# yanivw12/gs2mesh

Hardware: AMD Instinct MI355X
Metric: stereo-pair renders/sec + TSDF Mvoxel-updates/sec (higher is better)
Workload: dtype f32

## Files before the change

gs2mesh_amd/csrc/raster_api.hip:

```cpp
#include <stdarg.h>
#include <stdio.h>
#include <stdlib.h>
#include <string.h>

#include <string>
#include <vector>

#include "../../include/gs2mesh_amd.h"
#include "device_memory.h"
#include "raster_internal.h"

static thread_local std::string g_err;
void gs2m_set_error(const char* fmt, ...) {
    char buf[1024];
    va_list ap;
    va_start(ap, fmt);
    vsnprintf(buf, sizeof(buf), fmt, ap);
    va_end(ap);
    g_err = buf;
}
extern "C" const char* gs2m_last_error(void) { return g_err.c_str(); }
extern "C" int gs2m_version(void) { return GS2M_VERSION; }

#define GS2M_SORT_CLASSES_API 3
#define GS2M_MAX_STATUS 64

struct gs2m_raster {
    int device = 0;
    int opt_exact_cull = 0, opt_blend = 4, opt_debug = 0, opt_timing = 0, opt_tile_rows = 1, opt_pair_batch = 0;
    int opt_bin_workgroups = 256, opt_bin_wg_threads = 1024, opt_blend_mode = 2;
    int opt_blend_profile = 0;
    int opt_project_shared = 0;
    int opt_bin_lane_tiles = 4;
    DeviceBuffer<unsigned long long> d_blend_prof;
    EventPool events;
    DeviceBuffer<CamUniform> d_cams;
    DeviceBuffer<float4> d_recs;
    DeviceBuffer<unsigned long long> d_tilemask;
    DeviceBuffer<float> d_shpack;
    const float* pack_src = nullptr;
    const float* pack_src_rest = nullptr;
    int pack_P = 0;
    DeviceBuffer<float> d_pk_xyz, d_pk_scales, d_pk_rots, d_pk_opac;
    DeviceBuffer<int> d_order, d_rank;
    const float* model_src[4] = {nullptr, nullptr, nullptr, nullptr};
    bool model_packed = false;
    bool hint_valid = false;
    bool last_packed = false;
    const int* run_rank = nullptr;
    DeviceBuffer<unsigned> d_hist;
    DeviceBuffer<unsigned> d_tile_count, d_tile_start;
    DeviceBuffer<unsigned> d_sort_lists;
    DeviceBuffer<unsigned long long> d_keys, d_tmp;
    unsigned inst_cap = 0;
    DeviceBuffer<ViewStatus> d_status;
    PinnedBuffer<ViewStatus> h_status;
    DeviceBuffer<float> d_bw_rows;
    DeviceBuffer<unsigned> d_bw_offset;
    DeviceBuffer<unsigned> d_bw_blocks;
    DeviceBuffer<unsigned long long> d_bw_total;
    unsigned long long bw_last_rows = 0;
    bool fw_valid = false;
    int fw_P = 0, fw_W = 0, fw_H = 0, fw_tile_rows = 1;
    int last_P = 0, last_nv = 0, last_tiles = 0, last_views_total = 0;
    unsigned last_cap = 0;
};

extern "C" int gs2m_raster_create(gs2m_raster** out, int device) {
    if (!out) {
        gs2m_set_error("gs2m_raster_create: out is NULL");
        return 1;
    }
    GS2M_HIPCHK(hipSetDevice(device));
    gs2m_raster* r = new gs2m_raster();
    r->device = device;
    const size_t n_status = GS2M_MAX_STATUS + 1;
    if (r->d_cams.reserve_exact(GS2M_MAX_PASS_VIEWS) || r->d_status.reserve_exact(n_status) || r->h_status.reserve(n_status) ||
        hipMemset(r->d_status.get(), 0, sizeof(ViewStatus) * n_status) != hipSuccess) {
        gs2m_set_error("gs2m_raster_create: allocation failed");
        delete r;
        return 1;
    }
    memset(r->h_status.get(), 0, sizeof(ViewStatus) * n_status);
    *out = r;
    return 0;
}

extern "C" int gs2m_raster_destroy(gs2m_raster* r) {
    delete r;
    return 0;
}

extern "C" int gs2m_raster_set_option(gs2m_raster* r, int option, int value) {
    if (!r) {
        gs2m_set_error("null handle");
        return 1;
    }
    switch (option) {
        case GS2M_OPT_EXACT_TILE_CULL:
            if (value < 0 || value > 2) {
                gs2m_set_error("GS2M_OPT_EXACT_TILE_CULL must be 0, 1 or 2");
                return 1;
            }
            r->opt_exact_cull = value;
            return 0;
        case GS2M_OPT_BLEND_VARIANT:
            if (value != 0 && value != 4) {
                gs2m_set_error("GS2M_OPT_BLEND_VARIANT must be 0 or 4");
                return 1;
            }
            r->opt_blend = value;
            return 0;
        case GS2M_OPT_TILE_ROWS:
            if (value != 1 && value != 2) {
                gs2m_set_error("GS2M_OPT_TILE_ROWS must be 1 or 2");
                return 1;
// ... 95 lines not shown
        return 1;
    }
    if (instances > 0 && (unsigned)instances > r->inst_cap) r->inst_cap = (unsigned)instances;
    if (r->inst_cap < 1024) r->inst_cap = 1024;
    if (r->d_keys.reserve((size_t)nv * r->inst_cap)) return 1;
    if (r->d_tmp.reserve((size_t)nv * r->inst_cap)) return 1;
    return 0;
}

static int dbg_check(gs2m_raster* r, hipStream_t st, const char* what) {
    if (!r->opt_debug) return 0;
    hipError_t e = hipStreamSynchronize(st);
    if (e == hipSuccess) e = hipGetLastError();
    if (e != hipSuccess) {
        gs2m_set_error("[debug] after %s: %s", what, hipGetErrorString(e));
        return 1;
    }
    return 0;
}

static const char* const kStageRange[GS2M_N_STAGES] = {"gs2m:project", "gs2m:hist_colscan", "gs2m:tile_scan", "gs2m:scatter",
                                                        "gs2m:sort_tiles", "gs2m:blend", "gs2m:count_tiles"};
static StageTimer stage_timer(gs2m_raster* r, hipStream_t st, int stage) {
    return StageTimer(r->events, r->opt_timing != 0, st, stage, kStageRange[stage]);
}

static int run_views(gs2m_raster* r, const GaussIn& g, int nv, int pairs, int W, int H, float* out_color,
                     unsigned char* out_rgb8, int* out_radii, int status_slot, hipStream_t st, const CamUniform* host_cams) {
    const int nvt = nv * pairs;
    const int gx = (W + GS2M_TILE - 1) / GS2M_TILE, gy = (H + GS2M_TILE - 1) / GS2M_TILE;
    const int gys = (gy + r->opt_tile_rows - 1) / r->opt_tile_rows;
    const int tiles = gx * gys;
    int hint[3] = {-1, -1, -1};
    int interleave = 1;
    const ViewStatus* hs = r->h_status.get() + 1 + status_slot;
    if (r->hint_valid && r->last_tiles == tiles && r->last_nv == nvt) {
        unsigned nr_max = 0;
        for (int c = 0; c < 3; ++c) {
            unsigned m = 0;
            for (int v = 0; v < nvt; ++v) {
                const unsigned x = hs[v].n_class[c];
                m = x > m ? x : m;
            }
            hint[c] = m > 0x3fffffffu ? -1 : (int)m;
        }
        for (int v = 0; v < nvt; ++v) {
            const unsigned x = hs[v].num_rendered;
            nr_max = x > nr_max ? x : nr_max;
        }
        if (nr_max > 0u && nr_max <= 0x3fffffffu) interleave = (size_t)nr_max >= (size_t)800 * (size_t)tiles;
    }
    int chunk, n_wg;
    geometry(r, g.P, &chunk, &n_wg, pairs);
    int wg_threads = (gs2m_count_threads(chunk, r->opt_bin_wg_threads) + 63) / 64 * 64;
    while (wg_threads > 64 && (gs2m_scatter_lds_bytes(nv, tiles, wg_threads) > 160 * 1024 || gs2m_count_lds_bytes(nv, tiles, wg_threads) > 160 * 1024))
        wg_threads = (wg_threads / 2 + 63) / 64 * 64;
    const size_t lds = gs2m_scatter_lds_bytes(nv, tiles, wg_threads);
    const size_t lds_p = gs2m_count_lds_bytes(nv, tiles, wg_threads);
    if (lds > 160 * 1024 || lds_p > 160 * 1024) {
        gs2m_set_error("image %dx%d: %d views x %d tiles do not fit the 160 KiB LDS tile cursors", W, H, nv, tiles);
        return 1;
    }
    if (r->inst_cap == 0) {
        int64_t guess = (int64_t)g.P * 4;
        if (guess < 65536) guess = 65536;
        r->inst_cap = (unsigned)(guess > 0xfffffff0ll ? 0xfffffff0ll : guess);
    }
    if (gs2m_raster_reserve(r, g.P, nvt, W, H, 0)) return 1;
    const unsigned cap = r->inst_cap;
    const GeomRecs recs{r->d_recs.get(), r->d_recs.get() + 2 * (size_t)nvt * (size_t)g.P};
    const int cull_arg_p = r->opt_exact_cull, cull_arg_s = r->opt_exact_cull;
    {
        StageTimer tm = stage_timer(r, st, GS2M_STAGE_PROJECT);
        gs2m_launch_project(nv, pairs, st, g, r->d_cams.get(), recs, out_radii, cull_arg_p, host_cams, r->opt_project_shared);
    }
    if (dbg_check(r, st, "project")) return 1;
    {
        StageTimer tm = stage_timer(r, st, GS2M_STAGE_COUNT);
        if (gs2m_launch_count_tiles(nv, pairs, n_wg, wg_threads, lds_p, st, recs, g.P, r->d_cams.get(), chunk, r->d_hist.get(), r->d_tilemask.get(),
                                    cull_arg_p, g.ids != nullptr, r->opt_bin_lane_tiles))
            return 1;
    }
    if (dbg_check(r, st, "count_tiles")) return 1;
    {
        StageTimer tm = stage_timer(r, st, GS2M_STAGE_COLSCAN);
        gs2m_launch_hist_colscan(st, nvt, r->d_hist.get(), n_wg, tiles, r->d_tile_count.get());
    }
    if (dbg_check(r, st, "hist_colscan")) return 1;
    {
        StageTimer tm = stage_timer(r, st, GS2M_STAGE_TILESCAN);
        gs2m_launch_tile_scan(st, nvt, r->d_tile_count.get(), r->d_tile_start.get(), tiles, gx, r->h_status.get() + 1 + status_slot, r->d_status.get(), cap, r->d_sort_lists.get());
    }
    if (dbg_check(r, st, "tile_scan")) return 1;
    {
        StageTimer tm = stage_timer(r, st, GS2M_STAGE_SCATTER);
        if (gs2m_launch_scatter(nv, pairs, n_wg, wg_threads, lds, st, recs, g.P, r->d_cams.get(), chunk, r->d_hist.get(), r->d_tile_start.get(),
                                r->d_tilemask.get(), r->d_keys.get(), cap, cull_arg_s, g.ids, g.ids != nullptr, r->opt_bin_lane_tiles))
            return 1;
    }
    if (dbg_check(r, st, "scatter")) return 1;
    {
        StageTimer tm = stage_timer(r, st, GS2M_STAGE_SORT);
        gs2m_launch_sort_tiles(st, nvt, r->d_keys.get(), r->d_tmp.get(), r->d_tile_start.get(), tiles, cap, r->d_sort_lists.get(), hint);
    }
    if (dbg_check(r, st, "sort_tiles")) return 1;
    {
        StageTimer tm = stage_timer(r, st, GS2M_STAGE_BLEND);
        if (gs2m_launch_blend(st, r->opt_blend, r->opt_tile_rows, nvt, gx, gy, r->d_keys.get(), r->d_tile_start.get(), recs, r->d_cams.get(),
                              g.P, cap, out_color, out_rgb8, g.ids ? r->run_rank : nullptr,
                              r->d_sort_lists.get() + (size_t)nvt * GS2M_SORT_CLASSES_API * (tiles + 1), r->opt_blend_mode,
                              r->opt_blend_profile ? r->d_blend_prof.get() : nullptr, interleave))
            return 1;
    }
    if (dbg_check(r, st, "blend")) return 1;
    r->last_P = g.P;
    r->hint_valid = true;
    r->last_packed = g.ids != nullptr;
    r->last_nv = nvt;
    r->last_tiles = tiles;
    r->last_cap = cap;
    return 0;
}

extern "C" int gs2m_rasterize_forward(gs2m_raster* r, int P, int D, int M, const float* background, int width,
                                      int height, const float* means3D, const float* shs,
                                      const float* colors_precomp, const float* opacities, const float* scales,
                                      float scale_modifier, const float* rotations, const float* cov3D_precomp,
                                      const float* viewmatrix, const float* projmatrix, const float* cam_pos,
                                      float tan_fovx, float tan_fovy, int prefiltered, float* out_color,
                                      int* radii, int debug, gs2m_stream stream) {
    (void)prefiltered;
    if (!r) {
        gs2m_set_error("null handle");
        return 1;
    }
    hipStream_t st = (hipStream_t)stream;
    GS2M_HIPCHK(hipSetDevice(r->device));
    if (width <= 0 || height <= 0 || !out_color) {
        gs2m_set_error("gs2m_rasterize_forward: bad image arguments");
        return 1;
    }
    if (D < 0 || D > 3) {
        gs2m_set_error("SH degree %d not in 0..3", D);
        return 1;
    }
    r->last_views_total = 1;
    r->fw_valid = false;
    if (P == 0) {
        GS2M_HIPCHK(hipMemsetAsync(out_color, 0, sizeof(float) * 3 * (size_t)width * height, st));
// ... 539 lines not shown
```

gs2mesh_amd/csrc/raster_bin.hip:

```cpp
#include "raster_sort.h"
#include "raster_internal.h"

void gs2m_launch_hist_colscan(hipStream_t st, int nv, unsigned* hist, int n_wg, int tiles, unsigned* tile_count) {
    GS2M_LAUNCH(k_hist_colscan, dim3((tiles + 63) / 64, nv), dim3(64 * GS2M_COLSCAN_SEGS), 0, st, hist, n_wg, tiles, tile_count);
}
void gs2m_launch_tile_scan(hipStream_t st, int nv, const unsigned* tile_count, unsigned* tile_start, int tiles, int gx,
                           ViewStatus* status, ViewStatus* sticky, unsigned cap, unsigned* sort_lists) {
    GS2M_LAUNCH(k_tile_scan, dim3(nv), dim3(1024), 0, st, tile_count, tile_start, tiles, gx, status, sticky, cap, sort_lists);
}
size_t gs2m_sort_lists_words(int nv, int tiles) { return (size_t)nv * (GS2M_SORT_CLASSES * (tiles + 1) + tiles); }
void gs2m_launch_sort_tiles(hipStream_t st, int nv, unsigned long long* keys, unsigned long long* tmp,
                            const unsigned* tile_start, int tiles, unsigned cap, const unsigned* sort_lists, const int* class_hint) {
    const int fold = class_hint && class_hint[0] == 0 && class_hint[1] == 0 && class_hint[2] == 0;
    GS2M_LAUNCH(k_sort_tiles_small<4>, dim3((tiles + 3) / 4, nv), dim3(256), 0, st, keys, tile_start, tiles, cap, tmp, sort_lists, fold);
    if (fold) return;
    const int full[3] = {tiles < 1024 ? tiles : 1024, tiles < 512 ? tiles : 512, tiles < 512 ? tiles : 512};
    int g[3];
    for (int c = 0; c < 3; ++c) {
        g[c] = full[c];
        if (class_hint && class_hint[c] >= 0) {
            const int want = class_hint[c] + class_hint[c] / 2 + 16;
            g[c] = want < full[c] ? want : full[c];
        }
        if (g[c] < 1) g[c] = 1;
    }
    GS2M_LAUNCH(k_sort_tiles_bucket_4096x8, dim3(g[0], nv), dim3(512), 0, st, keys, tile_start, tiles, cap, sort_lists);
    GS2M_LAUNCH(k_sort_tiles_bucket_8192x8, dim3(g[1], nv), dim3(1024), 0, st, keys, tile_start, tiles, cap, sort_lists);
    GS2M_LAUNCH(k_sort_tiles, dim3(g[2], nv), dim3(256), 0, st, keys, tmp, tile_start, tiles, cap, sort_lists);
}
```

gs2mesh_amd/csrc/raster_blend.h:

```cpp
#pragma once
#include <type_traits>
#include "raster_common.h"

GS2M_DEVICE unsigned char quantize_u8(float c) {
    float v = rintf(c * 255.0f);
    v = fminf(255.0f, fmaxf(0.0f, v));
    return (unsigned char)(int)v;
}

GS2M_KERNEL void __launch_bounds__(256)
k_blend_tile256(const unsigned long long* __restrict__ keys, const unsigned* __restrict__ tile_start,
                const GeomRecs recs, const CamUniform* __restrict__ cams, int P, unsigned cap,
                float* __restrict__ out_color, unsigned char* __restrict__ out_rgb8, const int* __restrict__ rank) {
    __shared__ float4 s_a[256];
    __shared__ float4 s_b[256];
    __shared__ float s_c[256];
    const int v = (int)blockIdx.z;
    const CamUniform& cam = cams[v];
    const int W = cam.W, H = cam.H, gx = cam.gx;
    const int tiles = gx * cam.gy;
    const int tile = (int)blockIdx.y * gx + (int)blockIdx.x;
    const int tid = (int)threadIdx.x;
    const int lx = tid & 15, ly = tid >> 4;
    const int pxi = (int)blockIdx.x * GS2M_TILE + lx, pyi = (int)blockIdx.y * GS2M_TILE + ly;
// ... 407 lines not shown
            atomicAdd(&pc[5], pt_loop);
            atomicAdd(&pc[6], pt_epi);
            atomicAdd(&pc[7], pn_batches);
            atomicAdd(&pc[8], pn_staged);
            atomicAdd(&pc[9], (unsigned long long)(r1 - r0));
        }
    }
}

template <int LROWS>
GS2M_DEVICE bool blend_slot_tile(const CamUniform& cam, const unsigned* __restrict__ order, const int v, const int xcd, const int j,
                                 int& tx, int& ty) {
    const int gx = cam.gx;
    const int ltiles = gx * ((cam.gy + LROWS - 1) / LROWS);
    const int lrows = ltiles / gx, cpr = (gx + GS2M_SCHED_CW - 1) / GS2M_SCHED_CW;
    const int nch = cpr * ((lrows + GS2M_SCHED_CH - 1) / GS2M_SCHED_CH);
    const int rank_c = (j / (GS2M_SCHED_CHUNK * LROWS)) * 8 + xcd;
    if (rank_c >= nch) return false;
    const int c = (int)order[(size_t)v * ltiles + rank_c];
    const int k = (j / LROWS) % GS2M_SCHED_CHUNK;
    const int crow = c / cpr, lx = (c - crow * cpr) * GS2M_SCHED_CW + k % GS2M_SCHED_CW;
    const int ly = crow * GS2M_SCHED_CH + k / GS2M_SCHED_CW;
    if (lx >= gx || ly >= lrows) return false;
    tx = lx;
    ty = ly * LROWS + j % LROWS;
    return ty < cam.gy;
}

template <int WPB, int LROWS, int OCC, int MODE = 0, int PROF = 0>
GS2M_KERNEL void __launch_bounds__(64 * WPB, OCC)
k_blend_wave4e(const unsigned long long* __restrict__ keys, const unsigned* __restrict__ tile_start,
               const GeomRecs recs, const CamUniform* __restrict__ cams, int P, unsigned cap,
               float* __restrict__ out_color, unsigned char* __restrict__ out_rgb8, const int* __restrict__ rank,
               const unsigned* __restrict__ order, unsigned long long* __restrict__ prof = nullptr, int nv_x = 0) {
    __shared__ float4 s_a[WPB][64 + 2], s_b[WPB][64 + 2];
    __shared__ float2 s_c[WPB][64 + 2];
    __shared__ float4 s_raw[WPB][3 * 64];
    const int tid = (int)threadIdx.x;
    const int wave = tid >> 6, lane = tid & 63;
    const int nvx = gs2m_uniform(nv_x);
    const int v = nvx > 1 ? (int)((blockIdx.x / 8u) % (unsigned)nvx) : (int)blockIdx.y;
    const unsigned bid = nvx > 1 ? (blockIdx.x / 8u / (unsigned)nvx) * 8u + blockIdx.x % 8u : blockIdx.x;
    int tx, ty;
    if (!blend_slot_tile<LROWS>(cams[v], order, v, (int)(bid % 8u), gs2m_uniform((int)(bid / 8u) * WPB + wave), tx, ty)) return;
    blend_tile<WPB, LROWS, MODE, PROF>(v, tx, ty, cams[v], keys, tile_start, recs, P, cap, out_color, out_rgb8, rank, prof, &s_a[wave][0],
                                       &s_b[wave][0], &s_c[wave][0], &s_raw[wave][0], lane);
}
```

gs2mesh_amd/csrc/raster_blend.hip:

```cpp
#include "raster_blend.h"
#include "raster_backward_blend.h"
#include "raster_internal.h"

int gs2m_launch_blend(hipStream_t st, int variant, int tile_rows, int nv, int gx, int gy, const unsigned long long* keys,
                      const unsigned* tile_start, GeomRecs recs, const CamUniform* cams, int P, unsigned cap,
                      float* out_color, unsigned char* out_rgb8, const int* rank, const unsigned* order, int mode,
                      unsigned long long* prof, int interleave_views) {
    const dim3 block(256);
    if (variant == 4) {
        const int ltiles = gx * ((gy + tile_rows - 1) / tile_rows);
        const int nch = ((gx + GS2M_SCHED_CW - 1) / GS2M_SCHED_CW) * ((ltiles / gx + GS2M_SCHED_CH - 1) / GS2M_SCHED_CH);
        const dim3 g2(8u * ((unsigned)(((nch + 7) / 8) * GS2M_SCHED_CHUNK * tile_rows + 3) / 4u), nv);
        if (mode >= 2) {
            const int nvx = interleave_views && nv > 1 ? nv : 0;
            const dim3 g1 = nvx ? dim3(g2.x * (unsigned)nv, 1) : g2;
            if (prof) {
                if (tile_rows == 2) GS2M_LAUNCH((k_blend_wave4e<4, 2, 7, 2, 1>), g1, block, 0, st, keys, tile_start, recs, cams, P, cap, out_color, out_rgb8, rank, order, prof, nvx);
                else GS2M_LAUNCH((k_blend_wave4e<4, 1, 7, 2, 1>), g1, block, 0, st, keys, tile_start, recs, cams, P, cap, out_color, out_rgb8, rank, order, prof, nvx);
                return 0;
            }
            if (mode == 3) {
                if (tile_rows == 2) GS2M_LAUNCH((k_blend_wave4e<4, 2, 7, 3>), g1, block, 0, st, keys, tile_start, recs, cams, P, cap, out_color, out_rgb8, rank, order, nullptr, nvx);
                else GS2M_LAUNCH((k_blend_wave4e<4, 1, 7, 3>), g1, block, 0, st, keys, tile_start, recs, cams, P, cap, out_color, out_rgb8, rank, order, nullptr, nvx);
                return 0;
            }
            if (tile_rows == 2) GS2M_LAUNCH((k_blend_wave4e<4, 2, 7, 2>), g1, block, 0, st, keys, tile_start, recs, cams, P, cap, out_color, out_rgb8, rank, order, nullptr, nvx);
            else GS2M_LAUNCH((k_blend_wave4e<4, 1, 7, 2>), g1, block, 0, st, keys, tile_start, recs, cams, P, cap, out_color, out_rgb8, rank, order, nullptr, nvx);
            return 0;
        }
        if (tile_rows == 2) GS2M_LAUNCH((k_blend_wave4e<4, 2, 7>), g2, block, 0, st, keys, tile_start, recs, cams, P, cap, out_color, out_rgb8, rank, order, nullptr);
        else GS2M_LAUNCH((k_blend_wave4e<4, 1, 7>), g2, block, 0, st, keys, tile_start, recs, cams, P, cap, out_color, out_rgb8, rank, order, nullptr);
        return 0;
    }
    if (variant == 0 && tile_rows == 1) {
        GS2M_LAUNCH(k_blend_tile256, dim3(gx, gy, nv), dim3(256), 0, st, keys, tile_start, recs, cams, P, cap, out_color, out_rgb8, rank);
        return 0;
    }
    gs2m_set_error("blend variant %d is not available with GS2M_OPT_TILE_ROWS %d (variants: 0 [rows 1 only], 4)", variant, tile_rows);
    return 1;
}

void gs2m_launch_blend_backward(hipStream_t st, int gx, int gy, const unsigned long long* keys, const unsigned* tile_start,
                                GeomRecs recs, const CamUniform* cams, int P, unsigned cap, const float* dL_dpix,
                                const unsigned* row_offset, float* rows, unsigned long long n_rows) {
    const int tiles = gx * gy;
    GS2M_LAUNCH((k_blend_backward<4>), dim3((tiles + 3) / 4), dim3(256), 0, st, keys, tile_start, recs, cams, P, cap, dL_dpix,
                row_offset, rows, n_rows);
}
```

gs2mesh_amd/csrc/raster_common.h:

```cpp
#pragma once
#include "platform.h"

#define GS2M_TILE 16
#define GS2M_MAX_VIEWS 2
#define GS2M_MAX_PAIRS 4
#define GS2M_MAX_PASS_VIEWS (GS2M_MAX_VIEWS * GS2M_MAX_PAIRS)
#define GS2M_SORT_LDS 4096
#ifndef GS2M_SCHED_CW
#define GS2M_SCHED_CW 4
#endif
#ifndef GS2M_SCHED_CH
#define GS2M_SCHED_CH 2
#endif
#define GS2M_SCHED_CHUNK (GS2M_SCHED_CW * GS2M_SCHED_CH)
#define GS2M_BW_ROW 12

struct CamUniform {
    float view[16];
    float proj[16];
    float campos[3];
    float tanfovx, tanfovy, focal_x, focal_y;
    int W, H, gx, gy;
    float bg[3];
    int th;
// ... 6 lines not shown
    float cc, op, r, g;
    float b, depth;
    unsigned rect0, rect1;
};
struct GeomRecs {
    float4* ab;
    float4* c;
};
GS2M_DEVICE GeomRecs gs2m_recs_at(const GeomRecs& r, size_t first) { return GeomRecs{r.ab + 2 * first, r.c + first}; }

struct GaussIn {
    const float* xyz;
    const float* scales;
    const float* rots;
    const float* opac;
    const float* shs;
    const float* shs_rest;
    const float* shs_packed;
    const float* cov3D_precomp;
    const float* colors_precomp;
    const int* ids;
    int P, D, M, raw;
    float scale_modifier;
};

GS2M_DEVICE unsigned gs2m_xcd_contiguous(unsigned bid, unsigned nwg) {
    const unsigned qq = nwg / 8u, rr = nwg % 8u, xcd = bid % 8u, idx = bid / 8u;
    return (xcd < rr ? xcd * (qq + 1u) : rr * (qq + 1u) + (xcd - rr) * qq) + idx;
}

struct ViewStatus {
    unsigned num_rendered;
    unsigned overflow;
    unsigned n_class[3];
    unsigned pad;
};
```

gs2mesh_amd/csrc/raster_internal.h:

```cpp
#pragma once
#include "api_check.h"
#include "raster_common.h"

size_t gs2m_scatter_lds_bytes(int nv, int tiles, int threads);
void gs2m_launch_project(int nv, int pairs, hipStream_t st, const GaussIn& g, CamUniform* cams, GeomRecs recs, int* radii,
                         int exact_cull, const CamUniform* host_cams, int shared_read);
int gs2m_launch_count_tiles(int nv, int pairs, int n_wg, int threads, size_t lds_bytes, hipStream_t st, GeomRecs recs, int P,
                            const CamUniform* cams, int chunk, unsigned* hist, unsigned long long* tilemask,
                            int exact_cull, int interleave, int lane_tiles);
int gs2m_count_threads(int chunk, int max_threads);
size_t gs2m_count_lds_bytes(int nv, int tiles, int threads);
int gs2m_launch_scatter(int nv, int pairs, int n_wg, int threads, size_t lds_bytes, hipStream_t st, GeomRecs recs, int P,
                        const CamUniform* cams, int chunk, const unsigned* hist, const unsigned* tile_start,
                        const unsigned long long* tilemask, unsigned long long* keys, unsigned cap, int exact_cull,
                        const int* ids, int interleave, int lane_tiles);
void gs2m_launch_pack_sh(hipStream_t st, int P, const float* shs, const float* shs_rest, float* packed, const int* order);
void gs2m_launch_pack_model(hipStream_t st, int P, const int* order, const float* xyz, const float* scales, const float* rots,
                            const float* opac, float* p_xyz, float* p_scales, float* p_rots, float* p_opac, int* rank,
                            unsigned* bad);
void gs2m_launch_mark_visible(hipStream_t st, int P, const float* xyz, const float* viewmatrix,
                              unsigned char* present);
void gs2m_launch_pack_camera(hipStream_t st, CamUniform* cams, int slot, const float* viewmatrix,
                             const float* projmatrix, const float* campos, const float* bg, float tanfovx,
                             float tanfovy, int W, int H, int th);

void gs2m_launch_hist_colscan(hipStream_t st, int nv, unsigned* hist, int n_wg, int tiles, unsigned* tile_count);
void gs2m_launch_tile_scan(hipStream_t st, int nv, const unsigned* tile_count, unsigned* tile_start, int tiles, int gx,
                           ViewStatus* status, ViewStatus* sticky, unsigned cap, unsigned* sort_lists);
size_t gs2m_sort_lists_words(int nv, int tiles);
void gs2m_launch_sort_tiles(hipStream_t st, int nv, unsigned long long* keys, unsigned long long* tmp,
                            const unsigned* tile_start, int tiles, unsigned cap, const unsigned* sort_lists, const int* class_hint);
int gs2m_launch_blend(hipStream_t st, int variant, int tile_rows, int nv, int gx, int gy, const unsigned long long* keys,
                      const unsigned* tile_start, GeomRecs recs, const CamUniform* cams, int P,
                      unsigned cap, float* out_color, unsigned char* out_rgb8, const int* rank, const unsigned* order,
                      int mode, unsigned long long* prof, int interleave_views);

struct BwOut {
    float* dL_dmean2D;
    float* dL_dconic;
    float* dL_dopacity;
    float* dL_dcolor;
    float* dL_dmean3D;
    float* dL_dcov3D;
    float* dL_dsh;
    float* dL_dscale;
    float* dL_drot;
};
void gs2m_launch_bw_row_offsets(hipStream_t st, GeomRecs recs, int P, unsigned* block_sum, unsigned* row_offset,
                                unsigned long long* total_rows);
void gs2m_launch_blend_backward(hipStream_t st, int gx, int gy, const unsigned long long* keys, const unsigned* tile_start,
                                GeomRecs recs, const CamUniform* cams, int P, unsigned cap, const float* dL_dpix,
                                const unsigned* row_offset, float* rows, unsigned long long n_rows);
void gs2m_launch_gaussian_backward(hipStream_t st, const GaussIn& g, const CamUniform* cams, GeomRecs recs,
                                   const unsigned* row_offset, const float* rows, unsigned long long n_rows, const BwOut& out);
```

gs2mesh_amd/csrc/raster_sort.h:

```cpp
#pragma once
#include <type_traits>
#include "raster_common.h"

#define GS2M_SORT_WAVE 512
#define GS2M_SORT_CLASSES 3
#define GS2M_SORT_BUCKET_CAP 8192

#define GS2M_COLSCAN_SEGS 16
GS2M_KERNEL void __launch_bounds__(1024)
k_tile_scan(const unsigned* __restrict__ tile_count, unsigned* __restrict__ tile_start, int tiles, int gx,
            ViewStatus* __restrict__ status_all, ViewStatus* __restrict__ sticky, unsigned cap, unsigned* __restrict__ sort_lists) {
    const int v = (int)blockIdx.x, n_views = (int)gridDim.x;
    ViewStatus* status = status_all + v;
    __shared__ unsigned part[16];
    __shared__ unsigned n_class[GS2M_SORT_CLASSES];
    __shared__ unsigned w_pos[64];
    __shared__ unsigned w_max;
    const int tid = (int)threadIdx.x;
    const unsigned* cnt = tile_count + (size_t)v * tiles;
    unsigned* start = tile_start + (size_t)v * (tiles + 1);
    const int per = (tiles + 1023) / 1024;
    const int lo = tid * per;
    const int hi = lo + per < tiles ? lo + per : tiles;
    unsigned* lists = sort_lists + (size_t)v * GS2M_SORT_CLASSES * (tiles + 1);
    if (tid < GS2M_SORT_CLASSES) n_class[tid] = 0u;
    if (tid < 64) w_pos[tid] = 0u;
    if (tid == 64) w_max = 0u;
    __syncthreads();
    unsigned s = 0;
    for (int i = lo; i < hi; ++i) {
        const unsigned c = cnt[i];
        s += c;
        if (c > GS2M_SORT_WAVE) {
            const int cls = c <= 4096u ? 0 : (c <= GS2M_SORT_BUCKET_CAP ? 1 : 2);
            lists[cls * (tiles + 1) + 1 + atomicAdd(&n_class[cls], 1u)] = (unsigned)i;
        }
    }
    const int lane = tid & 63, wave = tid >> 6;
    unsigned incl = s;
#pragma unroll
    for (int d = 1; d < 64; d <<= 1) {
        const unsigned y = gs2m_shfl_up(incl, d);
        if (lane >= d) incl += y;
    }
// ... 27 lines not shown
    unsigned cw[2] = {0u, 0u};
    const bool sched = nch <= 2048;
    if (sched) {
        for (int k = 0; k < 2; ++k)
            if (tid + 1024 * k < nch) {
                cw[k] = chunk_weight(tid + 1024 * k);
                atomicMax(&w_max, cw[k]);
            }
    }
    __syncthreads();
    int wsh = 0;
    while ((w_max >> wsh) > 63u) ++wsh;
    if (sched)
        for (int k = 0; k < 2; ++k)
            if (tid + 1024 * k < nch) atomicAdd(&w_pos[63u - (cw[k] >> wsh)], 1u);
    __syncthreads();
    if (tid < 64) {
        const unsigned c = w_pos[tid];
        unsigned incl2 = c;
#pragma unroll
        for (int d = 1; d < 64; d <<= 1) {
            const unsigned y = gs2m_shfl_up(incl2, d);
            if (tid >= d) incl2 += y;
        }
        w_pos[tid] = incl2 - c;
    }
    __syncthreads();
    for (int k = 0; k < 2; ++k)
        if (tid + 1024 * k < nch) order[sched ? atomicAdd(&w_pos[63u - (cw[k] >> wsh)], 1u) : (unsigned)(tid + 1024 * k)] = (unsigned)(tid + 1024 * k);
    if (!sched)
        for (int c = tid + 2048; c < nch; c += 1024) order[c] = (unsigned)c;
    if (tid < GS2M_SORT_CLASSES) {
        lists[tid * (tiles + 1)] = n_class[tid];
        status->n_class[tid] = n_class[tid];
    }
    if (tid == 1023) {
        const unsigned total = total_all;
        start[tiles] = total;
        status->num_rendered = total;
        status->overflow = total > cap ? 1u : 0u;
        if (total > cap) atomicOr(&sticky->overflow, 1u);
        atomicMax(&sticky->num_rendered, total);
    }
}

GS2M_KERNEL void __launch_bounds__(64 * GS2M_COLSCAN_SEGS)
k_hist_colscan(unsigned* __restrict__ hist, int n_wg, int tiles, unsigned* __restrict__ tile_count) {
    __shared__ unsigned seg_sum[GS2M_COLSCAN_SEGS][64];
    const int lane = (int)(threadIdx.x & 63u), seg = (int)(threadIdx.x >> 6);
    const int t = (int)blockIdx.x * 64 + lane;
    const int v = (int)blockIdx.y;
    const int per = (n_wg + GS2M_COLSCAN_SEGS - 1) / GS2M_COLSCAN_SEGS;
    const int w0 = seg * per < n_wg ? seg * per : n_wg;
    const int w1 = w0 + per < n_wg ? w0 + per : n_wg;
    unsigned* col = hist + (size_t)v * n_wg * tiles + t;
    unsigned s = 0;
    if (t < tiles) {
        int w = w0;
        for (; w + 8 <= w1; w += 8) {
            unsigned x[8];
#pragma unroll
            for (int u = 0; u < 8; ++u) x[u] = col[(size_t)(w + u) * tiles];
#pragma unroll
            for (int u = 0; u < 8; ++u) s += x[u];
        }
        for (; w < w1; ++w) s += col[(size_t)w * tiles];
    }
    seg_sum[seg][lane] = s;
    __syncthreads();
    if (t < tiles) {
        unsigned run = 0, total = 0;
#pragma unroll
        for (int k = 0; k < GS2M_COLSCAN_SEGS; ++k) {
            const unsigned x = seg_sum[k][lane];
            run += k < seg ? x : 0u;
// ... 649 lines not shown
```

gs2mesh_amd/csrc/tsdf_api.hip:

```cpp
#include <math.h>
#include <stdio.h>
#include <string.h>

#include <mutex>
#include <vector>

#include "../../include/gs2mesh_amd.h"
#include "device_memory.h"
#include "tsdf_common.h"
#include "tsdf_internal.h"

struct gs2m_tsdf {
    int device = 0;
    double voxel_length = 0, sdf_trunc = 0, unit_length = 0;
    int color_type = 1, resolution = 16, stride = 4;
    TsdfVolume V;
    struct {
        DeviceBuffer<float> tsdf, weight;
        DeviceBuffer<unsigned> rgb, stamp, touched, counters;
        DeviceBuffer<int> block_keys, hash_vals;
        DeviceBuffer<unsigned char> halo;
        DeviceBuffer<unsigned long long> hash_keys, fmask, totals;
    } vol;
    unsigned frame_id = 0;
    PinnedBuffer<unsigned> h_counters;
    PinnedBuffer<unsigned long long> h_totals;
    int n_cu = 256;
    DeviceBuffer<unsigned char> d_mc;
    const McDevTables* mc() const { return reinterpret_cast<const McDevTables*>(d_mc.get()); }
    DeviceBuffer<unsigned> d_blk_tris;
    DeviceBuffer<unsigned long long> d_ntri;
    DeviceBuffer<double> mesh_v, mesh_c;
    DeviceBuffer<int> mesh_e;
    DeviceBuffer<int> mesh_tri;
    int64_t mesh_nv = 0, mesh_nt = 0;
    ScratchArena mesh_scratch;
    int timing = 0;
    EventPool events;
    DeviceBuffer<TsdfBatchFrame> d_bframes;
    static const int kRing = 8;
    PinnedBuffer<TsdfBatchFrame> h_bframes;
    hipEvent_t ring_done[8] = {nullptr, nullptr, nullptr, nullptr, nullptr, nullptr, nullptr, nullptr};
    unsigned ring_next = 0;
    ~gs2m_tsdf() {
        for (auto e : ring_done)
            if (e) (void)hipEventDestroy(e);
    }
};

static bool invert4x4(const double* m, double* inv) {
    double a[16];
    a[0] = m[5] * m[10] * m[15] - m[5] * m[11] * m[14] - m[9] * m[6] * m[15] + m[9] * m[7] * m[14] + m[13] * m[6] * m[11] - m[13] * m[7] * m[10];
    a[4] = -m[4] * m[10] * m[15] + m[4] * m[11] * m[14] + m[8] * m[6] * m[15] - m[8] * m[7] * m[14] - m[12] * m[6] * m[11] + m[12] * m[7] * m[10];
    a[8] = m[4] * m[9] * m[15] - m[4] * m[11] * m[13] - m[8] * m[5] * m[15] + m[8] * m[7] * m[13] + m[12] * m[5] * m[11] - m[12] * m[7] * m[9];
    a[12] = -m[4] * m[9] * m[14] + m[4] * m[10] * m[13] + m[8] * m[5] * m[14] - m[8] * m[6] * m[13] - m[12] * m[5] * m[10] + m[12] * m[6] * m[9];
    a[1] = -m[1] * m[10] * m[15] + m[1] * m[11] * m[14] + m[9] * m[2] * m[15] - m[9] * m[3] * m[14] - m[13] * m[2] * m[11] + m[13] * m[3] * m[10];
    a[5] = m[0] * m[10] * m[15] - m[0] * m[11] * m[14] - m[8] * m[2] * m[15] + m[8] * m[3] * m[14] + m[12] * m[2] * m[11] - m[12] * m[3] * m[10];
    a[9] = -m[0] * m[9] * m[15] + m[0] * m[11] * m[13] + m[8] * m[1] * m[15] - m[8] * m[3] * m[13] - m[12] * m[1] * m[11] + m[12] * m[3] * m[9];
    a[13] = m[0] * m[9] * m[14] - m[0] * m[10] * m[13] - m[8] * m[1] * m[14] + m[8] * m[2] * m[13] + m[12] * m[1] * m[10] - m[12] * m[2] * m[9];
    a[2] = m[1] * m[6] * m[15] - m[1] * m[7] * m[14] - m[5] * m[2] * m[15] + m[5] * m[3] * m[14] + m[13] * m[2] * m[7] - m[13] * m[3] * m[6];
    a[6] = -m[0] * m[6] * m[15] + m[0] * m[7] * m[14] + m[4] * m[2] * m[15] - m[4] * m[3] * m[14] - m[12] * m[2] * m[7] + m[12] * m[3] * m[6];
    a[10] = m[0] * m[5] * m[15] - m[0] * m[7] * m[13] - m[4] * m[1] * m[15] + m[4] * m[3] * m[13] + m[12] * m[1] * m[7] - m[12] * m[3] * m[5];
    a[14] = -m[0] * m[5] * m[14] + m[0] * m[6] * m[13] + m[4] * m[1] * m[14] - m[4] * m[2] * m[13] - m[12] * m[1] * m[6] + m[12] * m[2] * m[5];
    a[3] = -m[1] * m[6] * m[11] + m[1] * m[7] * m[10] + m[5] * m[2] * m[11] - m[5] * m[3] * m[10] - m[9] * m[2] * m[7] + m[9] * m[3] * m[6];
    a[7] = m[0] * m[6] * m[11] - m[0] * m[7] * m[10] - m[4] * m[2] * m[11] + m[4] * m[3] * m[10] + m[8] * m[2] * m[7] - m[8] * m[3] * m[6];
    a[11] = -m[0] * m[5] * m[11] + m[0] * m[7] * m[9] + m[4] * m[1] * m[11] - m[4] * m[3] * m[9] - m[8] * m[1] * m[7] + m[8] * m[3] * m[5];
    a[15] = m[0] * m[5] * m[10] - m[0] * m[6] * m[9] - m[4] * m[1] * m[10] + m[4] * m[2] * m[9] + m[8] * m[1] * m[6] - m[8] * m[2] * m[5];
    double det = m[0] * a[0] + m[1] * a[4] + m[2] * a[8] + m[3] * a[12];
    if (det == 0) return false;
    det = 1.0 / det;
    for (int i = 0; i < 16; i++) inv[i] = a[i] * det;
    return true;
}

static int zero_state(gs2m_tsdf* t, hipStream_t st, bool whole_pool, long long keep_first = -1) {
// ... 25 lines not shown
    while ((uint64_t)cap < 2ull * (uint64_t)max_blocks) cap <<= 1;
    V.hash_cap = cap;
    V.has_color = t->color_type == GS2M_TSDF_COLOR_RGB8;
    const size_t nvox = (size_t)max_blocks * GS2M_TSDF_VOX, nb = (size_t)max_blocks;
    auto& o = t->vol;
    if (o.tsdf.reserve_exact(nvox) || o.weight.reserve_exact(nvox) || (V.has_color && o.rgb.reserve_exact(3 * nvox)) ||
        o.block_keys.reserve_exact(3 * nb) || o.halo.reserve_exact(nb) || o.hash_keys.reserve_exact(cap) ||
        o.hash_vals.reserve_exact(cap) || o.stamp.reserve_exact(cap) || o.touched.reserve_exact(cap) || o.fmask.reserve_exact(cap) ||
        t->d_bframes.reserve_exact(GS2M_TSDF_MAX_BATCH) || t->h_bframes.reserve(GS2M_TSDF_MAX_BATCH * gs2m_tsdf::kRing) ||
        o.counters.reserve_exact(4) || o.totals.reserve_exact(1) || t->d_mc.reserve_exact(gs2m_mc_tables_bytes()) ||
        t->d_blk_tris.reserve_exact(nb) || t->d_ntri.reserve_exact(1) || t->h_counters.reserve(4) || t->h_totals.reserve(1)) {
        gs2m_set_error("gs2m_tsdf_create: out of device memory for %lld blocks (%.1f MiB)", (long long)max_blocks,
                       (double)nvox * 20.0 / 1048576.0);
        return 1;
    }
    V.tsdf = o.tsdf.get();
    V.weight = o.weight.get();
    V.rgb = o.rgb.get();
    V.block_keys = o.block_keys.get();
    V.halo = o.halo.get();
    V.hash_keys = o.hash_keys.get();
    V.hash_vals = o.hash_vals.get();
    V.stamp = o.stamp.get();
    V.touched = o.touched.get();
    V.fmask = o.fmask.get();
    V.counters = o.counters.get();
    V.totals = o.totals.get();
    std::vector<unsigned char> tab(gs2m_mc_tables_bytes());
    if (!gs2m_mc_tables_fill(tab.data()) ||
        hipMemcpy(t->d_mc.get(), tab.data(), tab.size(), hipMemcpyHostToDevice) != hipSuccess) {
        gs2m_set_error("gs2m_tsdf_create: marching-cubes table generation failed");
        return 1;
    }
    if (zero_state(t, (hipStream_t)0, true)) return 1;
    GS2M_HIPCHK(hipStreamSynchronize((hipStream_t)0));
    return 0;
}

extern "C" int gs2m_tsdf_create(gs2m_tsdf** out, double voxel_length, double sdf_trunc, int color_type,
                                int volume_unit_resolution, int depth_sampling_stride, int64_t max_blocks,
                                int device) {
    if (!out) {
        gs2m_set_error("gs2m_tsdf_create: out is NULL");
        return 1;
    }
    if (volume_unit_resolution != GS2M_TSDF_RES) {
        gs2m_set_error("volume_unit_resolution %d not supported (kernels are specialised for 16, Open3D's default)",
                       volume_unit_resolution);
        return 1;
    }
    if (!(voxel_length > 0) || !(sdf_trunc > 0) || depth_sampling_stride < 1 || max_blocks < 1 ||
        max_blocks > (1ll << 30) || (color_type != GS2M_TSDF_COLOR_NONE && color_type != GS2M_TSDF_COLOR_RGB8)) {
        gs2m_set_error("gs2m_tsdf_create: bad argument");
        return 1;
    }
    GS2M_HIPCHK(hipSetDevice(device));
    gs2m_tsdf* t = new gs2m_tsdf();
    t->device = device;
    t->voxel_length = voxel_length;
    t->sdf_trunc = sdf_trunc;
    t->unit_length = voxel_length * volume_unit_resolution;
    t->color_type = color_type;
    t->stride = depth_sampling_stride;
    if (init_volume(t, max_blocks)) {
        delete t;
        return 1;
// ... 95 lines not shown
        return 1;
    GS2M_HIPCHK(hipMemsetAsync(t->V.counters + 1, 0, sizeof(unsigned), st));
    {
        StageTimer tm(t->events, t->timing != 0, st, 0, "gs2m:tsdf_touch");
        gs2m_launch_tsdf_touch(st, t->V, f, depth, mask);
    }
    {
        StageTimer tm(t->events, t->timing != 0, st, 1, "gs2m:tsdf_integrate");
        gs2m_launch_tsdf_integrate(st, t->n_cu * 7, t->V, f, depth, color, mask);
    }
    return 0;
}

extern "C" int gs2m_tsdf_integrate_batch(gs2m_tsdf* t, int n_frames, const float* const* depth, const uint8_t* const* color,
                                         const uint8_t* const* mask, int width, int height, double fx, double fy, double cx,
                                         double cy, const double* extrinsics_w2c, double depth_scale, double depth_trunc,
                                         double min_depth, gs2m_stream stream) {
    if (!t || n_frames < 0 || (n_frames > 0 && (!depth || !extrinsics_w2c))) {
        gs2m_set_error("gs2m_tsdf_integrate_batch: NULL argument");
        return 1;
    }
    if (t->V.has_color && n_frames > 0 && !color) {
        gs2m_set_error("[ScalableTSDFVolume::Integrate] Unsupported image format.");
        return 1;
    }
    if (n_frames > 0 && check_frame_geometry("gs2m_tsdf_integrate_batch", width, height, fx, fy, depth_scale, 65535,
                                             " (the sweep packs pixel coordinates in 16 bits: <= 65535)"))
        return 1;
    GS2M_HIPCHK(hipSetDevice(t->device));
    hipStream_t st = (hipStream_t)stream;
    for (int f0 = 0; f0 < n_frames; f0 += GS2M_TSDF_MAX_BATCH) {
        const int nf = n_frames - f0 < GS2M_TSDF_MAX_BATCH ? n_frames - f0 : GS2M_TSDF_MAX_BATCH;
        const unsigned slot = t->ring_next++ % gs2m_tsdf::kRing;
        if (t->ring_done[slot]) GS2M_HIPCHK(hipEventSynchronize(t->ring_done[slot]));
        else GS2M_HIPCHK(hipEventCreateWithFlags(&t->ring_done[slot], hipEventDisableTiming));
        TsdfBatchFrame* hb = t->h_bframes.get() + (size_t)slot * GS2M_TSDF_MAX_BATCH;
        for (int k = 0; k < nf; ++k) {
            const int i = f0 + k;
            if (!depth[i] || (t->V.has_color && !color[i])) {
                gs2m_set_error("gs2m_tsdf_integrate_batch: frame %d has a NULL image", i);
                return 1;
            }
            const unsigned char* m = mask ? mask[i] : nullptr;
            if (fill_frame(t, hb[k].f, width, height, fx, fy, cx, cy, extrinsics_w2c + 16 * (size_t)i, depth_scale, depth_trunc,
                           min_depth, m != nullptr))
                return 1;
            hb[k].depth = depth[i];
            hb[k].color = color ? color[i] : nullptr;
            hb[k].mask = m;
        }
        GS2M_HIPCHK(hipMemcpyAsync(t->d_bframes.get(), hb, sizeof(TsdfBatchFrame) * nf, hipMemcpyHostToDevice, st));
        GS2M_HIPCHK(hipEventRecord(t->ring_done[slot], st));
        GS2M_HIPCHK(hipMemsetAsync(t->V.counters + 1, 0, sizeof(unsigned), st));
        GS2M_HIPCHK(hipMemsetAsync(t->V.counters + 3, 0, sizeof(unsigned), st));
        {
            StageTimer tm(t->events, t->timing != 0, st, 0, "gs2m:tsdf_touch_batch", nf);
            gs2m_launch_tsdf_touch_batch(st, t->V, hb[0].f, nf, t->d_bframes.get());
        }
        {
            StageTimer tm(t->events, t->timing != 0, st, 1, "gs2m:tsdf_integrate_batch", nf);
            gs2m_launch_tsdf_integrate_batch(st, t->n_cu, t->V, t->d_bframes.get());
        }
    }
    return 0;
}

extern "C" int gs2m_tsdf_set_stage_timing(gs2m_tsdf* t, int enable) {
    if (!t) {
// ... 458 lines not shown
```

Measured before the change: 4170.

## Move interleave decision to device and cache per-shape sort class hints

The blend kernel's choice between view-interleaved and per-view block ordering moves from a host decision, based on stale pinned status, to a device-written pass_order word set by the tile scan via atomicMax. Per-class sort-size hints are cached per (views, tiles) shape in an 8-entry LRU, so alternating image shapes no longer discard their hints. When no hint exists, the sort launch now sizes its grid as full/nv instead of full. TSDF ring events are created up front rather than lazily. The risk is that an undersized sort grid with no hint could starve work or become incorrect.

```diff
diff --git a/gs2mesh_amd/csrc/raster_api.hip b/gs2mesh_amd/csrc/raster_api.hip
--- a/gs2mesh_amd/csrc/raster_api.hip
+++ b/gs2mesh_amd/csrc/raster_api.hip
@@ -45,7 +45,6 @@
     DeviceBuffer<int> d_order, d_rank;
     const float* model_src[4] = {nullptr, nullptr, nullptr, nullptr};
     bool model_packed = false;
-    bool hint_valid = false;
     bool last_packed = false;
     const int* run_rank = nullptr;
     DeviceBuffer<unsigned> d_hist;
@@ -55,6 +54,15 @@
     unsigned inst_cap = 0;
     DeviceBuffer<ViewStatus> d_status;
     PinnedBuffer<ViewStatus> h_status;
+    struct HintShape {
+        int tiles = 0, views = 0;
+        unsigned long long used = 0;
+    };
+    HintShape hint_shape[GS2M_HINT_SHAPES];
+    unsigned long long hint_clock = 0;
+    PinnedBuffer<PassHint> h_hints;
+    DeviceBuffer<unsigned> d_pass_order;
+    unsigned pass_seq = 0;
     DeviceBuffer<float> d_bw_rows;
     DeviceBuffer<unsigned> d_bw_offset;
     DeviceBuffer<unsigned> d_bw_blocks;
@@ -74,14 +82,17 @@
     GS2M_HIPCHK(hipSetDevice(device));
     gs2m_raster* r = new gs2m_raster();
     r->device = device;
-    const size_t n_status = GS2M_MAX_STATUS + 1;
+    const size_t n_status = GS2M_MAX_STATUS + 1, n_hints = (size_t)GS2M_HINT_SHAPES * GS2M_MAX_PASS_VIEWS;
     if (r->d_cams.reserve_exact(GS2M_MAX_PASS_VIEWS) || r->d_status.reserve_exact(n_status) || r->h_status.reserve(n_status) ||
-        hipMemset(r->d_status.get(), 0, sizeof(ViewStatus) * n_status) != hipSuccess) {
+        r->h_hints.reserve(n_hints) || r->d_pass_order.reserve_exact(1) ||
+        hipMemset(r->d_status.get(), 0, sizeof(ViewStatus) * n_status) != hipSuccess ||
+        hipMemset(r->d_pass_order.get(), 0, sizeof(unsigned)) != hipSuccess) {
         gs2m_set_error("gs2m_raster_create: allocation failed");
         delete r;
         return 1;
     }
     memset(r->h_status.get(), 0, sizeof(ViewStatus) * n_status);
+    memset(r->h_hints.get(), 0xff, sizeof(PassHint) * n_hints);
     *out = r;
     return 0;
 }
@@ -243,10 +254,19 @@
     const int gys = (gy + r->opt_tile_rows - 1) / r->opt_tile_rows;
     const int tiles = gx * gys;
     int hint[3] = {-1, -1, -1};
-    int interleave = 1;
-    const ViewStatus* hs = r->h_status.get() + 1 + status_slot;
-    if (r->hint_valid && r->last_tiles == tiles && r->last_nv == nvt) {
-        unsigned nr_max = 0;
+    int shape = -1;
+    for (int i = 0; i < GS2M_HINT_SHAPES; ++i)
+        if (r->hint_shape[i].views == nvt && r->hint_shape[i].tiles == tiles) shape = i;
+    PassHint* const hints = r->h_hints.get();
+    if (shape < 0) {
+        shape = 0;
+        for (int i = 1; i < GS2M_HINT_SHAPES; ++i)
+            if (r->hint_shape[i].used < r->hint_shape[shape].used) shape = i;
+        r->hint_shape[shape].tiles = tiles;
+        r->hint_shape[shape].views = nvt;
+        memset(hints + (size_t)shape * GS2M_MAX_PASS_VIEWS, 0xff, sizeof(PassHint) * GS2M_MAX_PASS_VIEWS);
+    } else {
+        const PassHint* hs = hints + (size_t)shape * GS2M_MAX_PASS_VIEWS;
         for (int c = 0; c < 3; ++c) {
             unsigned m = 0;
             for (int v = 0; v < nvt; ++v) {
@@ -255,11 +275,11 @@
             }
             hint[c] = m > 0x3fffffffu ? -1 : (int)m;
         }
-        for (int v = 0; v < nvt; ++v) {
-            const unsigned x = hs[v].num_rendered;
-            nr_max = x > nr_max ? x : nr_max;
-        }
-        if (nr_max > 0u && nr_max <= 0x3fffffffu) interleave = (size_t)nr_max >= (size_t)800 * (size_t)tiles;
+    }
+    r->hint_shape[shape].used = ++r->hint_clock;
+    if (++r->pass_seq > 0x7ffffff0u) {
+        GS2M_HIPCHK(hipMemsetAsync(r->d_pass_order.get(), 0, sizeof(unsigned), st));
+        r->pass_seq = 1;
     }
     int chunk, n_wg;
     geometry(r, g.P, &chunk, &n_wg, pairs);
@@ -300,7 +320,8 @@
     if (dbg_check(r, st, "hist_colscan")) return 1;
     {
         StageTimer tm = stage_timer(r, st, GS2M_STAGE_TILESCAN);
-        gs2m_launch_tile_scan(st, nvt, r->d_tile_count.get(), r->d_tile_start.get(), tiles, gx, r->h_status.get() + 1 + status_slot, r->d_status.get(), cap, r->d_sort_lists.get());
+        gs2m_launch_tile_scan(st, nvt, r->d_tile_count.get(), r->d_tile_start.get(), tiles, gx, r->h_status.get() + 1 + status_slot, r->d_status.get(), cap, r->d_sort_lists.get(),
+                              hints + (size_t)shape * GS2M_MAX_PASS_VIEWS, r->d_pass_order.get(), r->pass_seq);
     }
     if (dbg_check(r, st, "tile_scan")) return 1;
     {
@@ -320,12 +341,11 @@
         if (gs2m_launch_blend(st, r->opt_blend, r->opt_tile_rows, nvt, gx, gy, r->d_keys.get(), r->d_tile_start.get(), recs, r->d_cams.get(),
                               g.P, cap, out_color, out_rgb8, g.ids ? r->run_rank : nullptr,
                               r->d_sort_lists.get() + (size_t)nvt * GS2M_SORT_CLASSES_API * (tiles + 1), r->opt_blend_mode,
-                              r->opt_blend_profile ? r->d_blend_prof.get() : nullptr, interleave))
+                              r->opt_blend_profile ? r->d_blend_prof.get() : nullptr, r->d_pass_order.get()))
             return 1;
     }
     if (dbg_check(r, st, "blend")) return 1;
     r->last_P = g.P;
-    r->hint_valid = true;
     r->last_packed = g.ids != nullptr;
     r->last_nv = nvt;
     r->last_tiles = tiles;
diff --git a/gs2mesh_amd/csrc/raster_bin.hip b/gs2mesh_amd/csrc/raster_bin.hip
--- a/gs2mesh_amd/csrc/raster_bin.hip
+++ b/gs2mesh_amd/csrc/raster_bin.hip
@@ -5,8 +5,10 @@
     GS2M_LAUNCH(k_hist_colscan, dim3((tiles + 63) / 64, nv), dim3(64 * GS2M_COLSCAN_SEGS), 0, st, hist, n_wg, tiles, tile_count);
 }
 void gs2m_launch_tile_scan(hipStream_t st, int nv, const unsigned* tile_count, unsigned* tile_start, int tiles, int gx,
-                           ViewStatus* status, ViewStatus* sticky, unsigned cap, unsigned* sort_lists) {
-    GS2M_LAUNCH(k_tile_scan, dim3(nv), dim3(1024), 0, st, tile_count, tile_start, tiles, gx, status, sticky, cap, sort_lists);
+                           ViewStatus* status, ViewStatus* sticky, unsigned cap, unsigned* sort_lists, PassHint* hint,
+                           unsigned* pass_order, unsigned pass_seq) {
+    GS2M_LAUNCH(k_tile_scan, dim3(nv), dim3(1024), 0, st, tile_count, tile_start, tiles, gx, status, sticky, cap, sort_lists, hint,
+                pass_order, pass_seq);
 }
 size_t gs2m_sort_lists_words(int nv, int tiles) { return (size_t)nv * (GS2M_SORT_CLASSES * (tiles + 1) + tiles); }
 void gs2m_launch_sort_tiles(hipStream_t st, int nv, unsigned long long* keys, unsigned long long* tmp,
@@ -17,7 +19,7 @@
     const int full[3] = {tiles < 1024 ? tiles : 1024, tiles < 512 ? tiles : 512, tiles < 512 ? tiles : 512};
     int g[3];
     for (int c = 0; c < 3; ++c) {
-        g[c] = full[c];
+        g[c] = full[c] / nv;
         if (class_hint && class_hint[c] >= 0) {
             const int want = class_hint[c] + class_hint[c] / 2 + 16;
             g[c] = want < full[c] ? want : full[c];
diff --git a/gs2mesh_amd/csrc/raster_blend.h b/gs2mesh_amd/csrc/raster_blend.h
--- a/gs2mesh_amd/csrc/raster_blend.h
+++ b/gs2mesh_amd/csrc/raster_blend.h
@@ -463,15 +463,26 @@
 k_blend_wave4e(const unsigned long long* __restrict__ keys, const unsigned* __restrict__ tile_start,
                const GeomRecs recs, const CamUniform* __restrict__ cams, int P, unsigned cap,
                float* __restrict__ out_color, unsigned char* __restrict__ out_rgb8, const int* __restrict__ rank,
-               const unsigned* __restrict__ order, unsigned long long* __restrict__ prof = nullptr, int nv_x = 0) {
+               const unsigned* __restrict__ order, unsigned long long* __restrict__ prof = nullptr, int nv_x = 0,
+               const unsigned* __restrict__ pass_order = nullptr) {
     __shared__ float4 s_a[WPB][64 + 2], s_b[WPB][64 + 2];
     __shared__ float2 s_c[WPB][64 + 2];
     __shared__ float4 s_raw[WPB][3 * 64];
     const int tid = (int)threadIdx.x;
     const int wave = tid >> 6, lane = tid & 63;
     const int nvx = gs2m_uniform(nv_x);
-    const int v = nvx > 1 ? (int)((blockIdx.x / 8u) % (unsigned)nvx) : (int)blockIdx.y;
-    const unsigned bid = nvx > 1 ? (blockIdx.x / 8u / (unsigned)nvx) * 8u + blockIdx.x % 8u : blockIdx.x;
+    int v = (int)blockIdx.y;
+    unsigned bid = blockIdx.x;
+    if (nvx > 1) {
+        if (gs2m_uniform((int)(*pass_order & 1u))) {
+            v = (int)((blockIdx.x / 8u) % (unsigned)nvx);
+            bid = (blockIdx.x / 8u / (unsigned)nvx) * 8u + blockIdx.x % 8u;
+        } else {
+            const unsigned per_view = gridDim.x / (unsigned)nvx;
+            v = (int)(blockIdx.x / per_view);
+            bid = blockIdx.x - (unsigned)v * per_view;
+        }
+    }
     int tx, ty;
     if (!blend_slot_tile<LROWS>(cams[v], order, v, (int)(bid % 8u), gs2m_uniform((int)(bid / 8u) * WPB + wave), tx, ty)) return;
     blend_tile<WPB, LROWS, MODE, PROF>(v, tx, ty, cams[v], keys, tile_start, recs, P, cap, out_color, out_rgb8, rank, prof, &s_a[wave][0],
diff --git a/gs2mesh_amd/csrc/raster_blend.hip b/gs2mesh_amd/csrc/raster_blend.hip
--- a/gs2mesh_amd/csrc/raster_blend.hip
+++ b/gs2mesh_amd/csrc/raster_blend.hip
@@ -5,27 +5,27 @@
 int gs2m_launch_blend(hipStream_t st, int variant, int tile_rows, int nv, int gx, int gy, const unsigned long long* keys,
                       const unsigned* tile_start, GeomRecs recs, const CamUniform* cams, int P, unsigned cap,
                       float* out_color, unsigned char* out_rgb8, const int* rank, const unsigned* order, int mode,
-                      unsigned long long* prof, int interleave_views) {
+                      unsigned long long* prof, const unsigned* pass_order) {
     const dim3 block(256);
     if (variant == 4) {
         const int ltiles = gx * ((gy + tile_rows - 1) / tile_rows);
         const int nch = ((gx + GS2M_SCHED_CW - 1) / GS2M_SCHED_CW) * ((ltiles / gx + GS2M_SCHED_CH - 1) / GS2M_SCHED_CH);
         const dim3 g2(8u * ((unsigned)(((nch + 7) / 8) * GS2M_SCHED_CHUNK * tile_rows + 3) / 4u), nv);
         if (mode >= 2) {
-            const int nvx = interleave_views && nv > 1 ? nv : 0;
+            const int nvx = nv > 1 ? nv : 0;
             const dim3 g1 = nvx ? dim3(g2.x * (unsigned)nv, 1) : g2;
             if (prof) {
-                if (tile_rows == 2) GS2M_LAUNCH((k_blend_wave4e<4, 2, 7, 2, 1>), g1, block, 0, st, keys, tile_start, recs, cams, P, cap, out_color, out_rgb8, rank, order, prof, nvx);
-                else GS2M_LAUNCH((k_blend_wave4e<4, 1, 7, 2, 1>), g1, block, 0, st, keys, tile_start, recs, cams, P, cap, out_color, out_rgb8, rank, order, prof, nvx);
+                if (tile_rows == 2) GS2M_LAUNCH((k_blend_wave4e<4, 2, 7, 2, 1>), g1, block, 0, st, keys, tile_start, recs, cams, P, cap, out_color, out_rgb8, rank, order, prof, nvx, pass_order);
+                else GS2M_LAUNCH((k_blend_wave4e<4, 1, 7, 2, 1>), g1, block, 0, st, keys, tile_start, recs, cams, P, cap, out_color, out_rgb8, rank, order, prof, nvx, pass_order);
                 return 0;
             }
             if (mode == 3) {
-                if (tile_rows == 2) GS2M_LAUNCH((k_blend_wave4e<4, 2, 7, 3>), g1, block, 0, st, keys, tile_start, recs, cams, P, cap, out_color, out_rgb8, rank, order, nullptr, nvx);
-                else GS2M_LAUNCH((k_blend_wave4e<4, 1, 7, 3>), g1, block, 0, st, keys, tile_start, recs, cams, P, cap, out_color, out_rgb8, rank, order, nullptr, nvx);
+                if (tile_rows == 2) GS2M_LAUNCH((k_blend_wave4e<4, 2, 7, 3>), g1, block, 0, st, keys, tile_start, recs, cams, P, cap, out_color, out_rgb8, rank, order, nullptr, nvx, pass_order);
+                else GS2M_LAUNCH((k_blend_wave4e<4, 1, 7, 3>), g1, block, 0, st, keys, tile_start, recs, cams, P, cap, out_color, out_rgb8, rank, order, nullptr, nvx, pass_order);
                 return 0;
             }
-            if (tile_rows == 2) GS2M_LAUNCH((k_blend_wave4e<4, 2, 7, 2>), g1, block, 0, st, keys, tile_start, recs, cams, P, cap, out_color, out_rgb8, rank, order, nullptr, nvx);
-            else GS2M_LAUNCH((k_blend_wave4e<4, 1, 7, 2>), g1, block, 0, st, keys, tile_start, recs, cams, P, cap, out_color, out_rgb8, rank, order, nullptr, nvx);
+            if (tile_rows == 2) GS2M_LAUNCH((k_blend_wave4e<4, 2, 7, 2>), g1, block, 0, st, keys, tile_start, recs, cams, P, cap, out_color, out_rgb8, rank, order, nullptr, nvx, pass_order);
+            else GS2M_LAUNCH((k_blend_wave4e<4, 1, 7, 2>), g1, block, 0, st, keys, tile_start, recs, cams, P, cap, out_color, out_rgb8, rank, order, nullptr, nvx, pass_order);
             return 0;
         }
         if (tile_rows == 2) GS2M_LAUNCH((k_blend_wave4e<4, 2, 7>), g2, block, 0, st, keys, tile_start, recs, cams, P, cap, out_color, out_rgb8, rank, order, nullptr);
diff --git a/gs2mesh_amd/csrc/raster_common.h b/gs2mesh_amd/csrc/raster_common.h
--- a/gs2mesh_amd/csrc/raster_common.h
+++ b/gs2mesh_amd/csrc/raster_common.h
@@ -62,6 +62,10 @@
 struct ViewStatus {
     unsigned num_rendered;
     unsigned overflow;
+};
+struct PassHint {
     unsigned n_class[3];
     unsigned pad;
 };
+#define GS2M_HINT_SHAPES 8
+#define GS2M_INTERLEAVE_MIN_PER_LIST 800u
diff --git a/gs2mesh_amd/csrc/raster_internal.h b/gs2mesh_amd/csrc/raster_internal.h
--- a/gs2mesh_amd/csrc/raster_internal.h
+++ b/gs2mesh_amd/csrc/raster_internal.h
@@ -26,14 +26,15 @@
 
 void gs2m_launch_hist_colscan(hipStream_t st, int nv, unsigned* hist, int n_wg, int tiles, unsigned* tile_count);
 void gs2m_launch_tile_scan(hipStream_t st, int nv, const unsigned* tile_count, unsigned* tile_start, int tiles, int gx,
-                           ViewStatus* status, ViewStatus* sticky, unsigned cap, unsigned* sort_lists);
+                           ViewStatus* status, ViewStatus* sticky, unsigned cap, unsigned* sort_lists, PassHint* hint,
+                           unsigned* pass_order, unsigned pass_seq);
 size_t gs2m_sort_lists_words(int nv, int tiles);
 void gs2m_launch_sort_tiles(hipStream_t st, int nv, unsigned long long* keys, unsigned long long* tmp,
                             const unsigned* tile_start, int tiles, unsigned cap, const unsigned* sort_lists, const int* class_hint);
 int gs2m_launch_blend(hipStream_t st, int variant, int tile_rows, int nv, int gx, int gy, const unsigned long long* keys,
                       const unsigned* tile_start, GeomRecs recs, const CamUniform* cams, int P,
                       unsigned cap, float* out_color, unsigned char* out_rgb8, const int* rank, const unsigned* order,
-                      int mode, unsigned long long* prof, int interleave_views);
+                      int mode, unsigned long long* prof, const unsigned* pass_order);
 
 struct BwOut {
     float* dL_dmean2D;
diff --git a/gs2mesh_amd/csrc/raster_sort.h b/gs2mesh_amd/csrc/raster_sort.h
--- a/gs2mesh_amd/csrc/raster_sort.h
+++ b/gs2mesh_amd/csrc/raster_sort.h
@@ -9,7 +9,8 @@
 #define GS2M_COLSCAN_SEGS 16
 GS2M_KERNEL void __launch_bounds__(1024)
 k_tile_scan(const unsigned* __restrict__ tile_count, unsigned* __restrict__ tile_start, int tiles, int gx,
-            ViewStatus* __restrict__ status_all, ViewStatus* __restrict__ sticky, unsigned cap, unsigned* __restrict__ sort_lists) {
+            ViewStatus* __restrict__ status_all, ViewStatus* __restrict__ sticky, unsigned cap, unsigned* __restrict__ sort_lists,
+            PassHint* __restrict__ hint, unsigned* __restrict__ pass_order, unsigned pass_seq) {
     const int v = (int)blockIdx.x, n_views = (int)gridDim.x;
     ViewStatus* status = status_all + v;
     __shared__ unsigned part[16];
@@ -103,7 +104,7 @@
         for (int c = tid + 2048; c < nch; c += 1024) order[c] = (unsigned)c;
     if (tid < GS2M_SORT_CLASSES) {
         lists[tid * (tiles + 1)] = n_class[tid];
-        status->n_class[tid] = n_class[tid];
+        hint[v].n_class[tid] = n_class[tid];
     }
     if (tid == 1023) {
         const unsigned total = total_all;
@@ -112,6 +113,8 @@
         status->overflow = total > cap ? 1u : 0u;
         if (total > cap) atomicOr(&sticky->overflow, 1u);
         atomicMax(&sticky->num_rendered, total);
+        const bool long_lists = (unsigned long long)total >= (unsigned long long)GS2M_INTERLEAVE_MIN_PER_LIST * (unsigned long long)tiles;
+        atomicMax(pass_order, 2u * pass_seq + (long_lists ? 1u : 0u));
     }
 }
 
diff --git a/gs2mesh_amd/csrc/tsdf_api.hip b/gs2mesh_amd/csrc/tsdf_api.hip
--- a/gs2mesh_amd/csrc/tsdf_api.hip
+++ b/gs2mesh_amd/csrc/tsdf_api.hip
@@ -40,7 +40,7 @@
     DeviceBuffer<TsdfBatchFrame> d_bframes;
     static const int kRing = 8;
     PinnedBuffer<TsdfBatchFrame> h_bframes;
-    hipEvent_t ring_done[8] = {nullptr, nullptr, nullptr, nullptr, nullptr, nullptr, nullptr, nullptr};
+    hipEvent_t ring_done[kRing] = {};
     unsigned ring_next = 0;
     ~gs2m_tsdf() {
         for (auto e : ring_done)
@@ -132,6 +132,7 @@
         gs2m_set_error("gs2m_tsdf_create: marching-cubes table generation failed");
         return 1;
     }
+    for (auto& e : t->ring_done) GS2M_HIPCHK(hipEventCreateWithFlags(&e, hipEventDisableTiming));
     if (zero_state(t, (hipStream_t)0, true)) return 1;
     GS2M_HIPCHK(hipStreamSynchronize((hipStream_t)0));
     return 0;
@@ -293,8 +294,7 @@
     for (int f0 = 0; f0 < n_frames; f0 += GS2M_TSDF_MAX_BATCH) {
         const int nf = n_frames - f0 < GS2M_TSDF_MAX_BATCH ? n_frames - f0 : GS2M_TSDF_MAX_BATCH;
         const unsigned slot = t->ring_next++ % gs2m_tsdf::kRing;
-        if (t->ring_done[slot]) GS2M_HIPCHK(hipEventSynchronize(t->ring_done[slot]));
-        else GS2M_HIPCHK(hipEventCreateWithFlags(&t->ring_done[slot], hipEventDisableTiming));
+        GS2M_HIPCHK(hipEventSynchronize(t->ring_done[slot]));
         TsdfBatchFrame* hb = t->h_bframes.get() + (size_t)slot * GS2M_TSDF_MAX_BATCH;
         for (int k = 0; k < nf; ++k) {
             const int i = f0 + k;
```

New measurement: 4169 (median of 2 runs). About the same (-0.0%).
